# DredderGun/accbpg_and_fw

Hardware: AMD Instinct MI355X
Metric: D-opt iters/sec (m=2048,n=32768) (higher is better)
Workload: dtype f64; 1 GPU; D_opt_design(2048,32768) abpg_gain gamma=2 fp64, one independent instance per GPU; instances=1, instances_per_gpu=1, seeds=1..1, window=transient: iterations 5..161 from x0 = 1/n, linear_gram=False

## Files before the change

### accbpg_and_fw_amd/csrc/capi.hip

```cpp
#include <stdarg.h>
#include <string.h>
#include <stdlib.h>
#include <algorithm>

#include "internal.h"
#include "reduce.hpp"
#include "trial_verdict.h"

namespace accbpg {

static thread_local char g_err[512] = "";

void set_last_error(const char* fmt, ...) {
    va_list ap;
    va_start(ap, fmt);
    vsnprintf(g_err, sizeof(g_err), fmt, ap);
    va_end(ap);
}

void note_tiles_fallback(const char* where) {
    static bool said = false;
    if (said) return;
    said = true;
    fprintf(stderr, "libaccbpg_hip: %s: the one-launch Cholesky abandoned a wait (another process on this GPU, or fewer "
// ... 526 lines not shown
        return accbpg_dopt_eval_gram(h, gram_dev, flag, f_host, g_dev);
    }
    if (fl[FLAG_NOT_PD]) {
        set_last_error("HXHT is singular or not positive definite");
        return ACCBPG_ERR_NOT_PD;
    }
    if (f_host) *f_host = -h->hpin[0];
    return ACCBPG_OK;
}

extern "C" int accbpg_dopt_profile_enable(accbpg_dopt* h, int enable) {
    if (!h) return ACCBPG_ERR_ARG;
    h->prof_on = enable != 0;
    return ACCBPG_OK;
}

extern "C" int accbpg_dopt_profile_reset(accbpg_dopt* h) {
    if (!h) return ACCBPG_ERR_ARG;
    ACC_HIP(hipStreamSynchronize(h->stream));
    for (auto& p : h->prof) { p.used = 0; p.total_ms = 0.0; p.launches = 0; }
    return ACCBPG_OK;
}

extern "C" int accbpg_dopt_profile_read(accbpg_dopt* h, int which, double* total_ms_host, int64_t* launches_host) {
    if (!h || which < 0 || which >= PROF_COUNT) return ACCBPG_ERR_ARG;
    ACC_HIP(hipStreamSynchronize(h->stream));
    ProfSlot& p = h->prof[which];
    double tot = 0.0;
    for (size_t i = 0; i + 1 < p.used; i += 2) {
        float ms = 0.f;
        ACC_HIP(hipEventElapsedTime(&ms, p.ev[i], p.ev[i + 1]));
        tot += ms;
    }
    p.total_ms = tot;
    if (total_ms_host) *total_ms_host = tot;
    if (launches_host) *launches_host = p.launches;
    return ACCBPG_OK;
}

extern "C" int accbpg_mfma_f64_peak(int iters, double* tflops_host, void* stream) {
    if (!tflops_host || iters <= 0) return ACCBPG_ERR_ARG;
    return mfma_peak(iters, tflops_host, (hipStream_t)stream);
}

extern "C" int accbpg_debug_pipe_probe(int iters, int mode, double* ms_host, void* stream) {
    if (!ms_host || iters <= 0) return ACCBPG_ERR_ARG;
    return pipe_probe(iters, mode, ms_host, (hipStream_t)stream);
}

extern "C" int accbpg_test_gemm(const double* A_dev, int64_t lda, const double* B_dev, int64_t ldb, double* C_dev,
                                int64_t ldc, int64_t M, int64_t N, int64_t K, int b_kmajor, double alpha,
                                double beta, int config, void* stream) {
    if (!A_dev || !B_dev || !C_dev || M <= 0 || N <= 0 || K <= 0) return ACCBPG_ERR_ARG;
    return launch_test_gemm(A_dev, lda, B_dev, ldb, C_dev, ldc, M, N, K, b_kmajor, alpha, beta, config,
                            (hipStream_t)stream);
}

extern "C" int accbpg_dopt_factor_in_small_launches(accbpg_dopt* h, int on) {
    if (!h || on < 0 || on > 2) return ACCBPG_ERR_ARG;
    const int64_t T = (h->m + NB - 1) / NB;
    value_forget(h);
    h->chol_tiles_off = on == 1 || (on == 2 && T * (T + 1) / 2 >= h->num_cu);
    return ACCBPG_OK;
}

extern "C" int accbpg_debug_plan_flags(int flags) {
    set_plan_flags(flags);
    return ACCBPG_OK;
}

extern "C" int accbpg_debug_gemm_loop(int variant) {
    return set_gemm_loop(variant);
}

extern "C" int accbpg_debug_chol_variant(accbpg_dopt* h, int bits) {
    if (!h) return ACCBPG_ERR_ARG;
    value_forget(h);
    h->chol_dbg = bits & 63;
    h->chol_tiles_off = (bits & 64) != 0;
    if (bits & 2048) h->chol_tiles_off = true;
    h->chol_stall_test = (bits & 128) ? 1 : 0;
    h->chol_spin_limit = (bits & 128) ? 200000 : 20000000;
    h->kern_variant = (bits >> 30) & 3;
    if (bits & 256) h->use_glds = false;
    if (bits & 512) h->use_glds = true;
    if (bits & 2048) {
        h->chol_two_level_T = (bits >> 12) & 0xfff;
        if ((bits >> 24) & 0x3f) h->chol_nk = (bits >> 24) & 0x3f;
    }
    return ACCBPG_OK;
}

extern "C" int accbpg_debug_chol_trace(accbpg_dopt* h, const double* gram_dev, int with_inverse, int64_t* stamps_host) {
    if (!h || !gram_dev || !stamps_host) return ACCBPG_ERR_ARG;
    if (!chol_tiles_usable(h)) {
        set_last_error("accbpg_debug_chol_trace: the one-launch Cholesky is not in use for this handle");
        return ACCBPG_ERR_ARG;
    }
    const int T = (int)((h->m + NB - 1) / NB);
    const size_t bytes = sizeof(long long) * (size_t)T * 32;
    if (!h->chol_trace) ACC_HIP(acc_malloc(&h->chol_trace, bytes, "chol_trace"));
    ACC_HIP(hipMemsetAsync(h->chol_trace, 0, bytes, h->stream));
    int rc = launch_cholesky(h, h->Lbuf, with_inverse ? h->Wbuf : nullptr, nullptr, gram_dev);
    if (rc == ACCBPG_OK) {
        hipError_t e = hipMemcpyAsync(stamps_host, h->chol_trace, bytes, hipMemcpyDeviceToHost, h->stream);
        if (e == hipSuccess) e = hipStreamSynchronize(h->stream);
        if (e != hipSuccess) rc = ACCBPG_ERR_HIP;
    }
    acc_free(h->chol_trace);
    h->chol_trace = nullptr;
    return rc;
}

extern "C" int accbpg_debug_gram_variant(accbpg_dopt* h, const double* x_dev, int variant, int iters, double* ms_host) {
    if (!h || !x_dev || !ms_host || iters <= 0) return ACCBPG_ERR_ARG;
    value_forget(h);
    return debug_gram_variant(h, x_dev, variant, iters, ms_host);
}

extern "C" int accbpg_debug_grad_variant(accbpg_dopt* h, double* g_dev, int variant, int iters, double* ms_host) {
    if (!h || !g_dev || !ms_host || iters <= 0) return ACCBPG_ERR_ARG;
    value_forget(h);
    return debug_grad_variant(h, g_dev, variant, iters, ms_host);
}
```

### accbpg_and_fw_amd/csrc/dopt_kernels.hip

```cpp
#include <atomic>
#include <mutex>
#include <type_traits>

#include "internal.h"
#include "mfma_tile.hpp"

namespace accbpg {

struct GramSeg {
    int64_t row0, col0, kb, ke;
    bool dual, whole;
};
template <class T>
__device__ __forceinline__ GramSeg gram_segment(const TileRC* __restrict__ tiles, int64_t kiters, int64_t it,
                                                int64_t it1) {
    const int e = (int)(it / kiters);
    const int64_t off = it - (int64_t)e * kiters;
    const TileRC tr = tiles[e];
    GramSeg g;
    if (tr.d1 < 0) {
        g.row0 = (int64_t)tr.rb * T::BM; g.col0 = (int64_t)tr.cb * T::BN;
        g.kb = off; g.ke = min(kiters, off + (it1 - it));
        g.dual = false;
        g.whole = (g.kb == 0 && g.ke == kiters);
// ... 84 lines not shown
    }
}

template <class T, int GV = 0>
__device__ __forceinline__ void gram_streamk_glds_body(
    const double* __restrict__ V, int64_t ldv, int64_t m, int64_t n, const double* __restrict__ x,
    const TileRC* __restrict__ tiles, const int64_t* __restrict__ wg_ranges, int64_t kiters, int nslot,
    double* __restrict__ slabs,
    double* __restrict__ G, int64_t ldg, int all_slabs) {
    extern __shared__ __attribute__((aligned(16))) double lds[];
    constexpr int NLD = T::G_NA + T::G_NB + 1;
    T t;
    int seg = 0;
    for (int rg = 0; rg < GRAM_RMAX; ++rg) {
    int64_t it = wg_ranges[((int64_t)blockIdx.x * GRAM_RMAX + rg) * 2];
    const int64_t it1 = wg_ranges[((int64_t)blockIdx.x * GRAM_RMAX + rg) * 2 + 1];
    while (it < it1) {
        const GramSeg sg = gram_segment<T>(tiles, kiters, it, it1);
        const int64_t kb = sg.kb, ke = sg.ke, row0 = sg.row0, col0 = sg.col0;
        const int64_t klast = ke - 1;
        t.zero();
        if constexpr (T::WAVES_N == 1) {
            if (sg.dual) {
                constexpr int NLDD = T::G_NLD_DUAL;
                const int64_t khalf = (kiters >> 1) * BK;
                t.glds_setup_A_dual(V, ldv, row0, khalf);
                __builtin_amdgcn_s_barrier();
                t.glds_issue_dual(kb * BK, x, khalf, lds);
                t.glds_issue_dual(min(kb + 1, klast) * BK, x, khalf, lds + T::G_STAGE);
                asm volatile("s_waitcnt vmcnt(%0)" ::"n"(NLDD) : "memory");
                __builtin_amdgcn_s_barrier();
                int cur = 0;
                t.template read_frag_dual<0>(lds, 0);
#pragma unroll 1
                for (int64_t ks = kb; ks < ke; ++ks) {
                    int nx2 = cur + 2;
                    if (nx2 >= 3) nx2 -= 3;
                    const double* st = lds + cur * T::G_STAGE;
                    t.template scale_dual<0>();
                    __builtin_amdgcn_sched_barrier(0);
                    t.template read_frag_dual<1>(st, 1);
                    __builtin_amdgcn_sched_barrier(0);
                    t.template mma_dual<0>();
                    t.glds_issue_dual(min(ks + 2, klast) * BK, x, khalf, lds + nx2 * T::G_STAGE);
                    __builtin_amdgcn_sched_barrier(0);
                    t.template scale_dual<1>();
                    __builtin_amdgcn_sched_barrier(0);
                    t.template read_frag_dual<0>(st, 2);
                    __builtin_amdgcn_sched_barrier(0);
                    t.template mma_dual<1>();
                    __builtin_amdgcn_sched_barrier(0);
                    t.template scale_dual<0>();
                    __builtin_amdgcn_sched_barrier(0);
                    t.template read_frag_dual<1>(st, 3);
                    __builtin_amdgcn_sched_barrier(0);
                    t.template mma_dual<0>();
                    __builtin_amdgcn_sched_barrier(0);
                    t.template scale_dual<1>();
                    __builtin_amdgcn_sched_barrier(0);
                    asm volatile("s_waitcnt vmcnt(%0)\n\ts_waitcnt lgkmcnt(0)" ::"n"(NLDD) : "memory");
                    __builtin_amdgcn_s_barrier();
                    cur = (cur + 1 == 3) ? 0 : cur + 1;
                    t.template read_frag_dual<0>(lds + cur * T::G_STAGE, 0);
                    __builtin_amdgcn_sched_barrier(0);
                    t.template mma_dual<1>();
                    __builtin_amdgcn_sched_barrier(0);
                }
                asm volatile("s_waitcnt vmcnt(0)\n\ts_waitcnt lgkmcnt(0)" ::: "memory");
                t.store_slab(slabs + ((int64_t)blockIdx.x * nslot + seg) * T::SLAB_DOUBLES);
                it += ke - kb;
                ++seg;
                continue;
            }
        }
        constexpr int PAIR = (GV & 256) ? 4 : (GV & 128) ? 2 : 1;
        t.template glds_setup_A<PAIR>(V, ldv, row0);
        t.template glds_setup_B_kc<PAIR>(V, ldv, col0);
        auto issue = [&](int64_t ks, int buf) {
            double* st = lds + buf * T::G_STAGE;
            t.template glds_issue<PAIR>(ks * BK, ks * BK, st);
            t.glds_x(x, ks * BK, st);
        };
        __builtin_amdgcn_s_barrier();
        issue(kb, 0);
        issue(min(kb + 1, klast), 1);
        asm volatile("s_waitcnt vmcnt(%0)" ::"n"(NLD) : "memory");
        __builtin_amdgcn_s_barrier();
        int cur = 0;
        t.template read_frag_g<0, true>(lds, 0);
        static_assert(T::MI == 4, "group 0 is dealt out over four fragment rows");
        constexpr int NP = T::G_NA + T::G_NB;
        constexpr int P1 = (NP + 2) / 3, P2 = 2 * P1 < NP ? 2 * P1 : NP;
        if constexpr (GV & 32) {
#pragma unroll 1
            for (int64_t ks = kb; ks < ke; ++ks) {
                int nx2 = cur + 2;
                if (nx2 >= 3) nx2 -= 3;
                int nx1 = cur + 1;
                if (nx1 >= 3) nx1 -= 3;
                const double* st = lds + cur * T::G_STAGE;
                const double* st1 = lds + nx1 * T::G_STAGE;
                double* nst = lds + nx2 * T::G_STAGE;
                const int64_t k2 = min(ks + 2, klast) * BK;
                auto group = [&](auto gtag) {
                    constexpr int g = decltype(gtag)::value;
                    constexpr int S = g & 1, NS = S ^ 1;
                    static_for<0, 16>([&](auto qtag) {
                        constexpr int q = decltype(qtag)::value;
                        constexpr int I = q >> 2, P = q & 3;
                        if constexpr (P == 0) t.template scale_row<S, I>();
                        __builtin_amdgcn_sched_barrier(0);
                        constexpr bool PB = (GV & 64) != 0;
                        constexpr int QBAR = PB ? 4 : 8;
                        if constexpr (g == 3 && q == QBAR && !(GV & 2)) {
                            if constexpr (GV & 8) asm volatile("s_waitcnt lgkmcnt(0)" ::: "memory");
                            else asm volatile("s_waitcnt vmcnt(%0)\n\ts_waitcnt lgkmcnt(0)" ::"n"(NLD) : "memory");
                            __builtin_amdgcn_s_barrier();
                        }
                        t.template mma_pair<S, I, P>();
                        __builtin_amdgcn_sched_barrier(0);
                        if constexpr (g < 3) {
                            constexpr int rp = PB ? q - 1 : (((q & 1) == 1) ? (q >> 1) : -1);
                            if constexpr (rp >= 0 && rp < 7 && !(GV & 4)) t.template read_part_g<NS, true, rp>(st, g + 1);
                            constexpr int lp = PB ? q - 8 : (((q & 1) == 0) ? (q >> 1) : -1);
                            if constexpr (g == 0 && lp >= 0 && !(GV & 1)) {
                                constexpr int p0 = 2 * lp;
                                if constexpr (PAIR == 4) {
                                    if constexpr (p0 < NP && p0 % 4 == 0) t.template glds_issue_range<4>(k2, k2, nst, p0, p0 + 4);
                                } else if constexpr (p0 < NP) t.template glds_issue_range<PAIR>(k2, k2, nst, p0, p0 + 2 < NP ? p0 + 2 : NP);
                                if constexpr (p0 == NP || (p0 + 1 == NP)) t.glds_x(x, k2, nst);
                            }
                        } else {
                            constexpr int rp = q - QBAR - (PB ? 1 : 0);
                            if constexpr (rp >= 0 && rp < 7 && !(GV & 4)) t.template read_part_g<NS, true, rp>(st1, 0);
                        }
                        __builtin_amdgcn_sched_barrier(0);
                    });
                };
                group(std::integral_constant<int, 0>{});
                group(std::integral_constant<int, 1>{});
                group(std::integral_constant<int, 2>{});
                group(std::integral_constant<int, 3>{});
                cur = nx1;
            }
        } else {
#pragma unroll 1
        for (int64_t ks = kb; ks < ke; ++ks) {
            int nx2 = cur + 2;
            if (nx2 >= 3) nx2 -= 3;
            const double* st = lds + cur * T::G_STAGE;
            double* nst = lds + nx2 * T::G_STAGE;
            const int64_t k2 = min(ks + 2, klast) * BK;
            t.template scale_frag<0>();
            __builtin_amdgcn_sched_barrier(0);
            if constexpr (!(GV & 4)) t.template read_frag_g<1, true>(st, 1);
            __builtin_amdgcn_sched_barrier(0);
            t.template mma_row<0>(0);
            if constexpr (!(GV & 1)) t.glds_issue_range(k2, k2, nst, 0, P1);
            t.template mma_row<0>(1);
            if constexpr (!(GV & 1)) t.glds_issue_range(k2, k2, nst, P1, P2);
            t.template mma_row<0>(2);
            if constexpr (!(GV & 1)) { t.glds_issue_range(k2, k2, nst, P2, NP); t.glds_x(x, k2, nst); }
            t.template mma_row<0>(3);
            __builtin_amdgcn_sched_barrier(0);
            t.template scale_frag<1>();
            __builtin_amdgcn_sched_barrier(0);
            if constexpr (!(GV & 4) && !(GV & 16)) t.template read_frag_g<0, true>(st, 2);
            __builtin_amdgcn_sched_barrier(0);
            t.template mma_frag<1>();
            __builtin_amdgcn_sched_barrier(0);
            t.template scale_frag<0>();
            __builtin_amdgcn_sched_barrier(0);
            if constexpr (!(GV & 4)) t.template read_frag_g<1, true>(st, 3);
            __builtin_amdgcn_sched_barrier(0);
            t.template mma_frag<0>();
            __builtin_amdgcn_sched_barrier(0);
            t.template scale_frag<1>();
            __builtin_amdgcn_sched_barrier(0);
            if constexpr (!(GV & 2)) {
                if constexpr (GV & 8) asm volatile("s_waitcnt lgkmcnt(0)" ::: "memory");
                else asm volatile("s_waitcnt vmcnt(%0)\n\ts_waitcnt lgkmcnt(0)" ::"n"(NLD) : "memory");
                __builtin_amdgcn_s_barrier();
            }
            cur = (cur + 1 == 3) ? 0 : cur + 1;
            if constexpr (!(GV & 4) && !(GV & 16)) t.template read_frag_g<0, true>(lds + cur * T::G_STAGE, 0);
            __builtin_amdgcn_sched_barrier(0);
            t.template mma_frag<1>();
            __builtin_amdgcn_sched_barrier(0);
        }
        }
        asm volatile("s_waitcnt vmcnt(0)\n\ts_waitcnt lgkmcnt(0)" ::: "memory");
        if (sg.whole && !all_slabs) {
            t.store_C(G, ldg, row0, col0, m, m, 1.0, 0.0, true);
        } else {
            t.store_slab(slabs + ((int64_t)blockIdx.x * nslot + seg) * T::SLAB_DOUBLES);
        }
        it += ke - kb;
        ++seg;
    }
    }
}

constexpr int GRAM_GV = 224;
template <class T, int GV = 0>
__global__ __launch_bounds__(NTHREADS, 1) void gram_streamk_glds_kernel(
    const double* __restrict__ V, int64_t ldv, int64_t m, int64_t n, const double* __restrict__ x,
    const TileRC* __restrict__ tiles, const int64_t* __restrict__ wg_ranges, int64_t kiters, int nslot,
    double* __restrict__ slabs,
    double* __restrict__ G, int64_t ldg, int all_slabs) {
    gram_streamk_glds_body<T, GV>(V, ldv, m, n, x, tiles, wg_ranges, kiters, nslot, slabs, G, ldg, all_slabs);
}
template <class T>
__global__ __launch_bounds__(NTHREADS, 1) void gram_streamk_glds_batch_kernel(
    const BatchInst* __restrict__ bt, BatchAct act, int64_t ldv, int64_t m, int64_t n, const double* __restrict__ xbase,
    int64_t ldx, const TileRC* __restrict__ tiles, const int64_t* __restrict__ wg_ranges, int64_t kiters, int nslot,
    int64_t ldg) {
    const int inst = act.idx[blockIdx.y];
    const BatchInst bi = bt[inst];
    gram_streamk_glds_body<T, GRAM_GV>(bi.V, ldv, m, n, xbase + (int64_t)inst * ldx, tiles, wg_ranges, kiters, nslot, bi.slabs,
                                       bi.gram, ldg, 0);
}

constexpr int FIX_PJ = 4;
template <class T>
__device__ __forceinline__ void gram_fixup_body(
    const TileRC* __restrict__ tiles, const int32_t* __restrict__ cstart, const int32_t* __restrict__ contrib,
    int nslot, const double* __restrict__ slabs, double* __restrict__ G, int64_t ldg, int64_t m, double beta) {
    constexpr int JW = (T::NI + FIX_PJ - 1) / FIX_PJ;
    const int jq = blockIdx.x % FIX_PJ;
    const int b = blockIdx.x / FIX_PJ;
    const int e = b / (2 * T::MI), hs = (b / T::MI) & 1, part = b % T::MI;
    const int j0 = jq * JW, j1 = min(T::NI, j0 + JW);
    if (j0 >= T::NI) return;
    const TileRC tr = tiles[e];
    const bool dual = tr.d1 >= 0;
    if (dual && part >= T::MI / 2) return;
    const int c0 = cstart[2 * e + hs], c1 = cstart[2 * e + hs + 1];
    if (c0 == c1) return;
    int64_t row0 = (int64_t)tr.rb * T::BM, col0 = (int64_t)tr.cb * T::BN;
    if (dual) row0 = col0 = (int64_t)(hs ? tr.d2 : tr.d1) * (T::BM / 2);
    if (col0 + 16 * j0 > row0 + 16 * (part * T::WAVES_M + T::WAVES_M - 1) + 15) return;
    double a[JW][4];
#pragma unroll
    for (int jj = 0; jj < JW; ++jj)
#pragma unroll
        for (int r = 0; r < 4; ++r) a[jj][r] = 0.0;
    const int tid = threadIdx.x;
    for (int c = c0; c < c1; ++c) {
        const int64_t w = contrib[2 * c];
        const int slot = contrib[2 * c + 1];
        const double* sl = slabs + (w * nslot + slot) * T::SLAB_DOUBLES;
#pragma unroll
        for (int jj = 0; jj < JW; ++jj) {
            const int j = j0 + jj;
            if (j < j1) {
#pragma unroll
                for (int r = 0; r < 4; ++r) {
                    a[jj][r] += sl[((part * T::NI + j) * 4 + r) * NTHREADS + tid];
                    if (dual) a[jj][r] += sl[(((part + T::MI / 2) * T::NI + j) * 4 + r) * NTHREADS + tid];
                }
            }
        }
    }
    const int lane = tid & 63, wave = tid >> 6;
    const int wm = wave / T::WAVES_N, wn = wave % T::WAVES_N;
    const int lr = lane & 15, lq = lane >> 4;
#pragma unroll
    for (int jj = 0; jj < JW; ++jj) {
        const int j = j0 + jj;
        if (j < j1) {
#pragma unroll
            for (int r = 0; r < 4; ++r) {
                const int rblk = dual ? T::dual_row_block(part, wm) : part * T::WAVES_M + wm;
                const int64_t row = row0 + 16 * rblk + lq + 4 * r;
                const int64_t col = col0 + wn * T::WN + 16 * j + lr;
                if (row < m && col < m && col <= row) {
                    double* gp = G + row * ldg + col;
                    *gp = (beta != 0.0) ? a[jj][r] + beta * *gp : a[jj][r];
                }
            }
        }
    }
}

template <class T>
__global__ __launch_bounds__(NTHREADS, 2) void gram_fixup_kernel(
// ... 1770 lines not shown
int build_plans(accbpg_dopt* h) {
    const int64_t m = h->m;
    GramPlanIn in;
    in.m = m; in.n = h->n; in.ldv = h->ldv;
    in.big = h->big; in.vec_ok = h->vec_ok; in.use_glds = h->use_glds;
    in.num_cu = h->num_cu; in.grid_cap = h->gram_grid_cap; in.flags = g_plan_flags;
    const GramPlan gp = plan_gram(in);
    if (!gp.ok) return ACCBPG_ERR_ARG;
    h->gram_chunks = gp.chunks;
    h->gram_nc = gp.nc;
    h->kiters = gp.kiters;
    h->has_duals = gp.has_duals;
    h->ntiles = (int)gp.tiles.size();
    h->gram_grid = gp.grid;
    h->gram_per = gp.per;
    h->gram_nslot = gp.nslot;
    if (gp.want_block_copy) {
        const size_t bytes = sizeof(double) * (size_t)m * (size_t)h->n;
        if (acc_malloc(&h->Vblk, bytes, "Vblk") == hipSuccess) {
            for (int c = 0; c < gp.chunks; ++c)
                ACC_HIP(hipMemcpy2DAsync(h->Vblk + (size_t)c * m * gp.nc, sizeof(double) * gp.nc,
                                         h->V + (size_t)c * gp.nc, sizeof(double) * (size_t)h->ldv,
                                         sizeof(double) * gp.nc, (size_t)m, hipMemcpyDeviceToDevice, h->stream));
            ACC_HIP(hipStreamSynchronize(h->stream));
        } else {
            (void)hipGetLastError();
            h->Vblk = nullptr;
        }
    }
    ACC_TRY(upload(gp.tiles, &h->tiles, "tiles"));
    ACC_TRY(upload(gp.ranges, &h->wg_ranges, "wg_ranges"));
    ACC_TRY(upload(gp.cstart, &h->gram_cstart, "gram_cstart"));
    ACC_TRY(upload(gp.contrib, &h->gram_contrib, "gram_contrib"));
    const size_t tile_doubles = h->big ? (size_t)TILE_BIG_M * TILE_BIG_N : (size_t)TILE_SMALL_M * TILE_SMALL_N;
    ACC_HIP(acc_malloc(&h->slabs, sizeof(double) * (size_t)gp.grid * gp.nslot * tile_doubles, "slabs"));

    ACC_HIP(acc_malloc(&h->Pbuf, sizeof(double) * (size_t)m * m, "Pbuf"));
    MergePlan mp = plan_merges(m, h->Lbuf, h->Wbuf, h->Tbuf, h->Pbuf);
    h->ops_host = std::move(mp.ops);
    h->red_host = std::move(mp.reds);
    h->merge_stages = std::move(mp.stages);
    ACC_TRY(upload(h->ops_host, &h->ops, "ops"));
    ACC_TRY(upload(h->red_host, &h->red, "red"));
    const int T = (int)((m + NB - 1) / NB);
    ACC_HIP(acc_malloc(&h->chol_op, sizeof(GemmOp) * (size_t)(T + 1), "chol_op"));

    if (T <= CT_TMAX) {
        const std::vector<CholJob> jobs = chol_jobs(T);
        ACC_TRY(ensure_lds(h->device, reinterpret_cast<const void*>(chol_tiles_kernel), CT_LDS_BYTES));
        int per_cu = 0;
        ACC_HIP(hipOccupancyMaxActiveBlocksPerMultiprocessor(&per_cu, chol_tiles_kernel, NTHREADS, CT_LDS_BYTES));
        h->chol_tiles_grid = (int)jobs.size();
        h->chol_slots = std::min(per_cu, 2) * h->num_cu;
        h->chol_tiles_ok = per_cu >= 1 && (int64_t)jobs.size() <= (int64_t)h->chol_slots;
        if (h->chol_tiles_ok) {
            CholJob* jobs_dev = nullptr;
            ACC_TRY(upload(jobs, &jobs_dev, "chol_jobs"));
            h->chol_jobs = jobs_dev;
            ACC_HIP(acc_malloc(&h->chol_ready, sizeof(int) * (size_t)(T * T + 5 * T), "chol_ready"));
            ACC_HIP(hipMemsetAsync(h->chol_ready, 0, sizeof(int) * (size_t)(T * T + 5 * T), h->stream));
            ACC_HIP(acc_malloc(&h->chol_hand, sizeof(double) * (size_t)T * NB * NB, "chol_hand"));
            ACC_HIP(acc_malloc(&h->chol_aux, sizeof(double) * (size_t)T * CT_AUX, "chol_aux"));
            ACC_HIP(acc_malloc(&h->Gbuf, sizeof(double) * (size_t)m * m, "Gbuf"));
            ACC_HIP(hipMemsetAsync(h->Gbuf, 0, sizeof(double) * (size_t)m * m, h->stream));
        }
    }
    ACC_HIP(hipStreamSynchronize(h->stream));
    return ACCBPG_OK;
}

template <class T>
static int gram_launch_t(accbpg_dopt* h, const double* x, double* gram) {
    if constexpr (!T::EDGE && T::BM == 256) {
        if (h->use_glds || h->has_duals) {
            const int64_t nc = h->gram_chunks > 1 ? h->gram_nc : h->n;
            for (int c = 0; c < h->gram_chunks; ++c) {
                const double* Vc = h->Vblk ? h->Vblk + (int64_t)c * h->m * nc : h->V + (int64_t)c * nc;
                const int64_t ldc = h->Vblk ? nc : h->ldv;
                const double* xc = x + (int64_t)c * nc;
                const double beta = c == 0 ? 0.0 : 1.0;
                const int all_slabs = h->gram_chunks > 1 ? 1 : 0;
                prof_begin(h, PROF_GRAM);
#define ACC_GRAM_ARGS Vc, ldc, h->m, nc, xc, h->tiles, h->wg_ranges, h->kiters, h->gram_nslot, h->slabs, gram, h->m, all_slabs
                if (h->kern_variant == 1)
                    ACC_LAUNCH_LDS(h->device, (gram_streamk_glds_kernel<T, GRAM_GV ^ 128>), h->gram_grid, NTHREADS, T::G_LDS_BYTES, h->stream, ACC_GRAM_ARGS);
                else if (h->kern_variant == 3)
                    ACC_LAUNCH_LDS(h->device, (gram_streamk_glds_kernel<T, 0>), h->gram_grid, NTHREADS, T::G_LDS_BYTES, h->stream, ACC_GRAM_ARGS);
                else if (h->kern_variant == 2)
                    ACC_LAUNCH_LDS(h->device, (gram_streamk_glds_kernel<T, (GRAM_GV ^ 128) | 256>), h->gram_grid, NTHREADS, T::G_LDS_BYTES, h->stream, ACC_GRAM_ARGS);
                else
                    ACC_LAUNCH_LDS(h->device, (gram_streamk_glds_kernel<T, GRAM_GV>), h->gram_grid, NTHREADS, T::G_LDS_BYTES, h->stream, ACC_GRAM_ARGS);
#undef ACC_GRAM_ARGS
                ACC_HIP(hipGetLastError());
                prof_end(h, PROF_GRAM);
                prof_begin(h, PROF_GRAMFIX);
                gram_fixup_kernel<T><<<h->ntiles * 2 * T::MI * FIX_PJ, NTHREADS, 0, h->stream>>>(
                    h->tiles, h->gram_cstart, h->gram_contrib, h->gram_nslot, h->slabs, gram, h->m, h->m, beta);
                prof_end(h, PROF_GRAMFIX);
            }
            return ACCBPG_OK;
        }
    }
    prof_begin(h, PROF_GRAM);
    ACC_LAUNCH_LDS(h->device, gram_streamk_kernel<T>, h->gram_grid, NTHREADS, T::LDS_BYTES, h->stream,
        h->V, h->ldv, h->m, h->n, x, h->tiles, h->wg_ranges, h->kiters, h->gram_nslot, h->slabs, gram, h->m, h->vec_ok);
    ACC_HIP(hipGetLastError());
    prof_end(h, PROF_GRAM);
    prof_begin(h, PROF_GRAMFIX);
    gram_fixup_kernel<T><<<h->ntiles * 2 * T::MI * FIX_PJ, NTHREADS, 0, h->stream>>>(h->tiles, h->gram_cstart, h->gram_contrib, h->gram_nslot,
                                                                h->slabs, gram, h->m, h->m, 0.0);
    prof_end(h, PROF_GRAMFIX);
    return ACCBPG_OK;
}

template <class F>
static int timed_launches(hipStream_t s, int iters, double* ms_out, F&& launch) {
    hipEvent_t a, b;
    ACC_HIP(hipEventCreate(&a));
    if (hipEventCreate(&b) != hipSuccess) {
        hipEventDestroy(a);
        return ACCBPG_ERR_HIP;
    }
    auto timed = [&]() -> int {
        ACC_TRY(launch());
        ACC_HIP(hipEventRecord(a, s));
        for (int i = 0; i < iters; ++i) ACC_TRY(launch());
        ACC_HIP(hipEventRecord(b, s));
        ACC_HIP(hipEventSynchronize(b));
        float ms = 0.f;
        ACC_HIP(hipEventElapsedTime(&ms, a, b));
        *ms_out = ms / iters;
        ACC_HIP(hipGetLastError());
        return ACCBPG_OK;
    };
    const int rc = timed();
    hipEventDestroy(a);
    hipEventDestroy(b);
    return rc;
}

int debug_gram_variant(accbpg_dopt* h, const double* x, int var, int iters, double* ms_out) {
    using T = TileBig<false, false>;
    if (!h->big) return ACCBPG_ERR_ARG;
    if (h->has_duals && var < 10) return ACCBPG_ERR_ARG;
    auto launch = [&]() -> int {
#define ACC_LAUNCH_VAR(VV)                                                                                       \
    ACC_LAUNCH_LDS(h->device, (gram_streamk_kernel<T, VV>), h->gram_grid, NTHREADS, T::LDS_BYTES, h->stream,      \
        h->V, h->ldv, h->m, h->n, x, h->tiles, h->wg_ranges, h->kiters, h->gram_nslot, h->slabs, h->Tbuf, h->m, h->vec_ok)
#define ACC_LAUNCH_G(GG)                                                                                         \
    ACC_LAUNCH_LDS(h->device, (gram_streamk_glds_kernel<T, GG>), h->gram_grid, NTHREADS, T::G_LDS_BYTES, h->stream,          \
        h->V, h->ldv, h->m, h->n, x, h->tiles, h->wg_ranges, h->kiters, h->gram_nslot, h->slabs, h->Tbuf, h->m, 0)
        switch (var) {
            case 10: ACC_LAUNCH_G(0); break;
            case 11: ACC_LAUNCH_G(1); break;
            case 12: ACC_LAUNCH_G(2); break;
            case 13: ACC_LAUNCH_G(3); break;
            case 14: ACC_LAUNCH_G(4); break;
            case 15: ACC_LAUNCH_G(8); break;
            case 16: ACC_LAUNCH_G(7); break;
            case 17: ACC_LAUNCH_G(16); break;
            case 18: ACC_LAUNCH_G(32); break;
            case 19: ACC_LAUNCH_G(96); break;
            case 20: ACC_LAUNCH_G(97); break;
            case 21: ACC_LAUNCH_G(98); break;
            case 22: ACC_LAUNCH_G(100); break;
            case 23: ACC_LAUNCH_G(104); break;
            case 24: ACC_LAUNCH_G(103); break;
            case 25: ACC_LAUNCH_G(102); break;
            case 26: ACC_LAUNCH_G(101); break;
            case 27: ACC_LAUNCH_G(99); break;
            case 28: ACC_LAUNCH_G(224); break;
            case 29: ACC_LAUNCH_G(352); break;
            case 0: ACC_LAUNCH_VAR(0); break;
            case 1: ACC_LAUNCH_VAR(1); break;
            case 2: ACC_LAUNCH_VAR(2); break;
            case 3: ACC_LAUNCH_VAR(3); break;
            default: ACC_LAUNCH_VAR(4); break;
        }
#undef ACC_LAUNCH_VAR
        return ACCBPG_OK;
    };
    return timed_launches(h->stream, iters, ms_out, launch);
}

int launch_gram(accbpg_dopt* h, const double* x, double* gram) {
    bool xal = (reinterpret_cast<uintptr_t>(x) & 15) == 0;
    if (!xal && (h->has_duals || h->gram_chunks > 1)) {
        if (!h->xbuf) ACC_HIP(acc_malloc(&h->xbuf, sizeof(double) * (size_t)h->n, "xbuf"));
        ACC_TRY(device_copy(h->xbuf, x, (size_t)h->n, h->stream));
        x = h->xbuf;
        xal = true;
    }
    if (h->big) {
        const bool interior = h->vec_ok && xal && (h->m % 256 == 0) && (h->n % BK == 0);
        if (interior) ACC_TRY((gram_launch_t<TileBig<false, false>>(h, x, gram)));
        else ACC_TRY((gram_launch_t<TileBig<false, true>>(h, x, gram)));
    } else {
        const bool interior = h->vec_ok && xal && (h->m % 64 == 0) && (h->n % BK == 0);
        if (interior) ACC_TRY((gram_launch_t<TileSmall<false, false>>(h, x, gram)));
        else ACC_TRY((gram_launch_t<TileSmall<false, true>>(h, x, gram)));
    }
    ACC_HIP(hipGetLastError());
    return ACCBPG_OK;
}

__global__ __launch_bounds__(256) void copy_kernel(double* __restrict__ dst, const double* __restrict__ src, size_t n) {
    const size_t stride = (size_t)gridDim.x * 256;
    for (size_t i = (size_t)blockIdx.x * 256 + threadIdx.x; i < n; i += stride) dst[i] = src[i];
}
int device_copy(double* dst, const double* src, size_t ndoubles, hipStream_t s) {
    if (ndoubles == 0 || dst == src) return ACCBPG_OK;
    size_t nb = (ndoubles + 255) / 256;
    if (nb > 4096) nb = 4096;
    copy_kernel<<<(unsigned)nb, 256, 0, s>>>(dst, src, ndoubles);
    ACC_HIP(hipGetLastError());
    return ACCBPG_OK;
}

int launch_gemm_ops(const GemmOp* ops_dev, int nops, int maxM, int maxN, bool b_kmajor, hipStream_t s) {
    if (nops <= 0 || maxM <= 0 || maxN <= 0) return ACCBPG_OK;
    dim3 grid((maxN + 63) / 64, (maxM + 63) / 64, nops);
    int dev = 0;
    ACC_HIP(hipGetDevice(&dev));
    return with_gemm_loop([&](auto loop) -> int {
        constexpr int LOOP = decltype(loop)::value;
        if (b_kmajor)
            ACC_LAUNCH_LDS(dev, (gemm_ops_kernel<TileSmall<true>, LOOP>), grid, NTHREADS, TileSmall<true>::LDS_BYTES, s, ops_dev);
        else
            ACC_LAUNCH_LDS(dev, (gemm_ops_kernel<TileSmall<false>, LOOP>), grid, NTHREADS, TileSmall<false>::LDS_BYTES, s, ops_dev);
        ACC_HIP(hipGetLastError());
        return ACCBPG_OK;
    });
}

static std::mutex g_tiles_mu;
constexpr int TILES_RING = 16;
struct TilesRing {
    hipEvent_t ev[TILES_RING] = {};
    hipStream_t stream[TILES_RING] = {};
    int grid[TILES_RING] = {};
    long long issued = 0;
};
static TilesRing g_tiles[64];

bool chol_tiles_usable(const accbpg_dopt* h) {
    return h->chol_tiles_ok && !h->chol_tiles_off && (h->chol_dbg & 63) == 0;
}

static int launch_chol_tiles(accbpg_dopt* h, const double* src, double* A, double* Winv, double* dscal, int* dflag) {
    const int64_t m = h->m;
    const int T = (int)((m + NB - 1) / NB);
    CholInst ci;
    ci.src = src; ci.L = A; ci.Ldiag = h->Tbuf; ci.Winv = Winv; ci.logdet = dscal; ci.flags = dflag;
    ci.ready = h->chol_ready; ci.aux = h->chol_aux; ci.hand = h->chol_hand; ci.trace = h->chol_trace;
    const int dev = (h->device >= 0 && h->device < 64) ? h->device : 0;
// ... 326 lines not shown
```

### accbpg_and_fw_amd/csrc/internal.h

```cpp
#pragma once
#include <hip/hip_runtime.h>
#include <stdint.h>
#include <stdio.h>
#include <map>
#include <mutex>
#include <utility>
#include <vector>

#include "../../include/accbpg_hip.h"
#include "dopt_plan.hpp"

namespace accbpg {

void set_last_error(const char* fmt, ...);
void note_tiles_fallback(const char* where);

hipError_t acc_malloc(void** p, size_t bytes, const char* label);
hipError_t acc_free(void* p);
template <class T>
inline hipError_t acc_malloc(T** p, size_t bytes, const char* label) {
    return acc_malloc(reinterpret_cast<void**>(p), bytes, label);
}

#define ACC_HIP(call)                                                                         \
// ... 163 lines not shown
constexpr int STATUS_DOUBLES = 20;
constexpr int ACCBPG_RETRY = 100;

enum ProfKind { PROF_GRAM = 0, PROF_CHOL = 1, PROF_TRTRI = 2, PROF_GRAD = 3, PROF_GRAMFIX = 4, PROF_FWV = 5, PROF_COUNT = 6 };

struct ProfSlot {
    std::vector<hipEvent_t> ev;
    size_t used = 0;
    double total_ms = 0.0;
    int64_t launches = 0;
};

}

struct accbpg_dopt {
    const double* V = nullptr;
    int64_t m = 0, n = 0, ldv = 0;
    hipStream_t stream = nullptr;
    int device = 0;
    int num_cu = 256;
    bool big = false;
    bool force_big = false;
    int gram_grid_cap = 0;
    double* dscal_ext = nullptr;
    bool vec_ok = false;

    double* Lbuf = nullptr;
    double* Wbuf = nullptr;
    double* Tbuf = nullptr;
    double* slabs = nullptr;
    accbpg::TileRC* tiles = nullptr;
    int64_t* wg_ranges = nullptr;
    int32_t* gram_cstart = nullptr;
    int32_t* gram_contrib = nullptr;
    int ntiles = 0, gram_grid = 0, gram_per = 0, gram_nslot = 2;
    int64_t kiters = 0;
    int gram_chunks = 1;
    int64_t gram_nc = 0;
    double* Vblk = nullptr;
    double* dscal = nullptr;
    int* dflag = nullptr;
    double* hpin = nullptr;
    double* vws = nullptr;
    double* xbuf = nullptr;

    accbpg::GemmOp* ops = nullptr;
    std::vector<accbpg::GemmOp> ops_host;
    std::vector<accbpg::RedOp> red_host;
    using MergeStage = accbpg::MergeStage;
    std::vector<MergeStage> merge_stages;
    accbpg::RedOp* red = nullptr;
    double* Pbuf = nullptr;
    accbpg::GemmOp* chol_op = nullptr;

    double *fw_x = nullptr, *fw_w = nullptr, *fw_H = nullptr, *fw_hv = nullptr;
    double* fw_hpin_dev = nullptr;
    accbpg::FwInst fw{};
    bool fw_ready = false;
    struct FwSlot {
        accbpg_dopt* aux = nullptr;
        hipStream_t stream = nullptr;
        hipEvent_t ev_snap = nullptr;
        bool pending = false;
    };
    std::vector<FwSlot> fw_ring;
    int fw_ring_depth = 1;
    int fw_ring_small = 2;
    long long fw_ring_issued = 0, fw_ring_collected = 0;
    int fw_part_nblk = 0;
    bool fw_part_away = false;
    accbpg::FwRunSlot* fw_run = nullptr;
    accbpg_fw_step* fw_steps_pin = nullptr;
    accbpg_fw_step* fw_steps_dev = nullptr;
    double* fw_div_ws = nullptr;
    double* fw_div_pin = nullptr;
    double* fw_div_pin_dev = nullptr;
    int64_t fw_div_i = -1;
    accbpg::FwDivRunSlot* fw_div_run = nullptr;
    accbpg_fw_div_step* fw_div_steps_pin = nullptr;
    accbpg_fw_div_step* fw_div_steps_dev = nullptr;

    bool use_glds = true;
    int kern_variant = 0;
    bool diag_inv_ready = false;
    bool has_duals = false;
    int chol_nk = 8;
    int chol_two_level_T = 64;
    int chol_dbg = 0;
    bool chol_tiles_ok = false;
    bool chol_tiles_off = false;
    int chol_stall_test = 0;
    long long chol_spin_limit = 20000000;
    int chol_tiles_grid = 0;
    int chol_slots = 0;
    void* chol_jobs = nullptr;
    int* chol_ready = nullptr;
    double* chol_aux = nullptr;
    double* chol_hand = nullptr;
    long long* chol_trace = nullptr;
    double* Gbuf = nullptr;
    const double* last_x = nullptr;
    double* last_g = nullptr;
    int last_flag = 0;
    hipEvent_t ev_done = nullptr;
    bool val_reuse = true;
    bool val_valid = false;
    bool val_pending = false;
    bool val_hit = false;
    const double* val_x = nullptr;
    double* val_copy = nullptr;
    double val_f = 0.0;
    double val_answer = 0.0;
    int val_gen = 0;
    int64_t val_compares = 0, val_answered = 0;
    double* trial_stat = nullptr;
    double* trial_pin = nullptr;
    accbpg_dopt* val_peer = nullptr;
    std::vector<accbpg_dopt*> val_linked;
    bool prof_on = false;
    accbpg::ProfSlot prof[accbpg::PROF_COUNT];
};

struct accbpg_dopt_batch {
    int K = 0;
    std::vector<accbpg_dopt*> inst;
    hipStream_t stream = nullptr;
    int device = 0;
    bool fast = false;
    int chunk = 0;
    accbpg::BatchInst* table = nullptr;
    accbpg::CholInst* chol_table[2] = {nullptr, nullptr};
    accbpg::GemmOp* ops_all = nullptr;
    accbpg::RedOp* red_all = nullptr;
    int ops_per_inst = 0, red_per_inst = 0;
    double* dscal_all = nullptr;
    double* hpin = nullptr;
    int* vflags = nullptr;
    double* vout = nullptr;
    double* vpart = nullptr;
    double* vws = nullptr;
    double* vquot = nullptr;
    double* vpin = nullptr;
    accbpg::FwInst* fw_table = nullptr;
    accbpg::FwDivInst* fw_div_table = nullptr;
    accbpg::FwRunSlot* fw_runs = nullptr;
    accbpg_fw_step* fw_bsteps_pin = nullptr;
    accbpg_fw_step* fw_bsteps_dev = nullptr;
    accbpg::FwDivRunSlot* fw_div_runs = nullptr;
    accbpg_fw_div_step* fw_div_bsteps_pin = nullptr;
    accbpg_fw_div_step* fw_div_bsteps_dev = nullptr;
    accbpg::BatchAct pend_act;
    const double* pend_x = nullptr;
    double* pend_g = nullptr;
    int64_t pend_ldx = 0, pend_ldg = 0;
    int pend_flag = 0;
    bool pend_fused = false;
};
struct BatchVals { double v[accbpg::BATCH_MAX]; };

namespace accbpg {

int launch_gram_batch(accbpg_dopt_batch* b, const BatchAct& act, const double* xbase, int64_t ldx);
int launch_cholesky_batch(accbpg_dopt_batch* b, const BatchAct& act, bool with_inverse, const double* xbase, int64_t ldx);
int launch_trtri_batch(accbpg_dopt_batch* b, const BatchAct& act);
int launch_colnorm_batch(accbpg_dopt_batch* b, const BatchAct& act, double* gbase, int64_t ldg, double sign);

// ... 44 lines not shown
```

### accbpg_and_fw_amd/csrc/mfma_tile.hpp

```cpp
#pragma once
#include <hip/hip_runtime.h>
#include <stdint.h>
#include <type_traits>

#include "dopt_plan.hpp"

namespace accbpg {

typedef double d4 __attribute__((ext_vector_type(4)));
typedef double d2 __attribute__((ext_vector_type(2)));

constexpr int SK = BK + 2;
constexpr int NTHREADS = 256;

typedef const __attribute__((address_space(1))) double* gptr;
__device__ __forceinline__ gptr as_global(const double* p) { return (gptr)p; }
__device__ __forceinline__ d2 ld2(const double* p) { return *reinterpret_cast<const d2*>(p); }
__device__ __forceinline__ d2 ld2(gptr p) { return *(const __attribute__((address_space(1))) d2*)p; }

template <class P>
__device__ __forceinline__ d2 load2_guard(P p, bool row_ok, int64_t k, int64_t K, bool vec_ok) {
    d2 v;
    if (row_ok && vec_ok && k + 1 < K) {
        v = ld2(p);
// ... 320 lines not shown
                        constexpr int pb = p - G_NA;
                        if constexpr (NPK == 2) glds16_run2<pb * 1024>(bb, gob[pb], gob[pb + 1], lb);
                        else glds16_run4<pb * 1024>(bb, gob[pb], gob[pb + 1], gob[pb + 2], gob[pb + 3], lb);
                    }
                }
            });
            return;
        }
#pragma unroll
        for (int p = 0; p < G_NA + G_NB; ++p)
            if (p >= p0 && p < p1) {
                uint32_t o = (p < G_NA) ? goa[p < G_NA ? p : 0] : gob[p >= G_NA ? p - G_NA : 0];
                asm volatile("" : "+v"(o));
                const char* b = (p < G_NA) ? ba : bb;
                glds16(reinterpret_cast<const double*>(b + o), stage + (p < G_NA ? 0 : G_A) + (wave + 4 * (p < G_NA ? p : p - G_NA)) * 128);
            }
    }
    __device__ __forceinline__ void glds_x(const double* __restrict__ x, int64_t k0, double* __restrict__ stage) const {
        const int lane = threadIdx.x & 63;
        const float* src = reinterpret_cast<const float*>(x + k0) + (lane & 31);
        __builtin_amdgcn_global_load_lds((const __attribute__((address_space(1))) void*)src,
                                         (__attribute__((address_space(3))) void*)(stage + G_A + G_B), 4, 0, 0);
    }
    template <int SET, bool SCALE>
    __device__ __forceinline__ void read_frag_g(const double* __restrict__ stage, int kk) {
        const int lane = threadIdx.x & 63, wave = __builtin_amdgcn_readfirstlane(threadIdx.x >> 6);
        const int wm = wave / WAVES_N, wn = wave % WAVES_N;
        const int lr = lane & 15, lq = lane >> 4;
        const int sw = (lr >> 1) & 7;
        const int koff = 2 * ((2 * kk + (lq >> 1)) ^ sw) + (lq & 1);
        const double* as = stage + (16 * wm + lr) * BK + koff;
#pragma unroll
        for (int i = 0; i < MI; ++i) fa[SET][i] = as[i * 16 * WAVES_M * BK];
        if constexpr (BKM) {
            const double* bs = stage + G_A + (4 * kk + lq) * BN + wn * WN + lr;
#pragma unroll
            for (int j = 0; j < NI; ++j) fb[SET][j] = bs[16 * (j ^ (lq & 1))];
        } else {
            const double* bs = stage + G_A + (wn * WN + lr) * BK + koff;
#pragma unroll
            for (int j = 0; j < NI; ++j) fb[SET][j] = bs[j * 16 * BK];
        }
        if constexpr (SCALE) fx[SET] = stage[G_A + G_B + 4 * kk + lq];
    }

    template <int SET, bool SCALE, int PART>
    __device__ __forceinline__ void read_part_g(const double* __restrict__ stage, int kk) {
        static_assert(MI == 4 && NI == 8, "parts are laid out for the 64 x 128 wave tile");
        const int lane = threadIdx.x & 63, wave = __builtin_amdgcn_readfirstlane(threadIdx.x >> 6);
        const int wm = wave / WAVES_N, wn = wave % WAVES_N;
        const int lr = lane & 15, lq = lane >> 4;
        const int sw = (lr >> 1) & 7;
        const int koff = 2 * ((2 * kk + (lq >> 1)) ^ sw) + (lq & 1);
        if constexpr (PART == 0) {
            if constexpr (SCALE) fx[SET] = stage[G_A + G_B + 4 * kk + lq];
        } else if constexpr (PART == 1 || PART == 6) {
            const double* as = stage + (16 * wm + lr) * BK + koff;
            constexpr int i0 = (PART == 1) ? 0 : 2;
            fa[SET][i0] = as[i0 * 16 * WAVES_M * BK];
            fa[SET][i0 + 1] = as[(i0 + 1) * 16 * WAVES_M * BK];
        } else {
            constexpr int j0 = 2 * (PART - 2);
            if constexpr (BKM) {
                const double* bs = stage + G_A + (4 * kk + lq) * BN + wn * WN + lr;
                fb[SET][j0] = bs[16 * (j0 ^ (lq & 1))];
                fb[SET][j0 + 1] = bs[16 * ((j0 + 1) ^ (lq & 1))];
            } else {
                const double* bs = stage + G_A + (wn * WN + lr) * BK + koff;
                fb[SET][j0] = bs[j0 * 16 * BK];
                fb[SET][j0 + 1] = bs[(j0 + 1) * 16 * BK];
            }
        }
    }
    template <int SET, int I>
    __device__ __forceinline__ void scale_row() { fa[SET][I] *= fx[SET]; }
    template <int SET, int I, int P>
    __device__ __forceinline__ void mma_pair(int mi_lo = 0) {
        if (I >= mi_lo) {
            acc[I][2 * P] = __builtin_amdgcn_mfma_f64_16x16x4f64(fa[SET][I], fb[SET][2 * P], acc[I][2 * P], 0, 0, 0);
            acc[I][2 * P + 1] = __builtin_amdgcn_mfma_f64_16x16x4f64(fa[SET][I], fb[SET][2 * P + 1], acc[I][2 * P + 1], 0, 0, 0);
        }
    }

    template <int SET, int ILO>
    __device__ __forceinline__ void read_frag_lo(const double* __restrict__ stage, int kk) {
        static_assert(BKM, "the gradient product reads a k-major B image");
        const int lane = threadIdx.x & 63, wave = __builtin_amdgcn_readfirstlane(threadIdx.x >> 6);
        const int wm = wave / WAVES_N, wn = wave % WAVES_N;
        const int lr = lane & 15, lq = lane >> 4;
        const int sw = (lr >> 1) & 7;
        const int koff = 2 * ((2 * kk + (lq >> 1)) ^ sw) + (lq & 1);
        const double* as = stage + (16 * wm + lr) * BK + koff;
#pragma unroll
        for (int i = ILO; i < MI; ++i) fa[SET][i] = as[i * 16 * WAVES_M * BK];
        const double* bs = stage + G_A + (4 * kk + lq) * BN + wn * WN + lr;
#pragma unroll
        for (int j = 0; j < NI; ++j) fb[SET][j] = bs[16 * (j ^ (lq & 1))];
    }
    template <int SET, int I, int ILO, bool COND>
    __device__ __forceinline__ void mma_row_lo(bool live) {
        if constexpr (I >= ILO) {
            if (!(COND && I == ILO) || live) {
#pragma unroll
                for (int j = 0; j < NI; ++j)
                    acc[I][j] = __builtin_amdgcn_mfma_f64_16x16x4f64(fa[SET][I], fb[SET][j], acc[I][j], 0, 0, 0);
            }
        }
    }
    template <int SET, int ILO, bool COND>
    __device__ __forceinline__ void mma_frag_lo(bool live) {
        static_assert(MI == 4, "four fragment rows");
        mma_row_lo<SET, 0, ILO, COND>(live);
        mma_row_lo<SET, 1, ILO, COND>(live);
        mma_row_lo<SET, 2, ILO, COND>(live);
        mma_row_lo<SET, 3, ILO, COND>(live);
    }
    template <int RUN, int ILO, int ILO_NEXT, bool COND, int NLD, int AB = 0>
    __device__ __forceinline__ void grad_step(const double* __restrict__ st, const double* __restrict__ st1,
                                              double* __restrict__ nst, int64_t ka, int64_t kb, bool live) {
        constexpr int NP = G_NA + G_NB;
        constexpr int P1 = (NP + 2) / 3, P2 = 2 * P1 < NP ? 2 * P1 : NP;
        static_assert(NLD == NP, "every wave retires the loads of one step per step");
        if constexpr (!(AB & 4)) read_frag_lo<1, ILO>(st, 1);
        __builtin_amdgcn_sched_barrier(0);
        mma_row_lo<0, 0, ILO, COND>(live);
        if constexpr (!(AB & 1)) glds_issue_range<RUN>(ka, kb, nst, 0, P1);
        mma_row_lo<0, 1, ILO, COND>(live);
        if constexpr (!(AB & 1)) glds_issue_range<RUN>(ka, kb, nst, P1, P2);
        mma_row_lo<0, 2, ILO, COND>(live);
        if constexpr (!(AB & 1)) glds_issue_range<RUN>(ka, kb, nst, P2, NP);
        mma_row_lo<0, 3, ILO, COND>(live);
        __builtin_amdgcn_sched_barrier(0);
        if constexpr (!(AB & 4)) read_frag_lo<0, ILO>(st, 2);
        __builtin_amdgcn_sched_barrier(0);
        mma_frag_lo<1, ILO, COND>(live);
        __builtin_amdgcn_sched_barrier(0);
        if constexpr (!(AB & 4)) read_frag_lo<1, ILO>(st, 3);
        __builtin_amdgcn_sched_barrier(0);
        mma_frag_lo<0, ILO, COND>(live);
        __builtin_amdgcn_sched_barrier(0);
        if constexpr (!(AB & 2)) {
            asm volatile("s_waitcnt vmcnt(%0)\n\ts_waitcnt lgkmcnt(0)" ::"n"(NLD) : "memory");
            __builtin_amdgcn_s_barrier();
        }
        if constexpr (!(AB & 4)) read_frag_lo<0, ILO_NEXT>(st1, 0);
        __builtin_amdgcn_sched_barrier(0);
        mma_frag_lo<1, ILO, COND>(live);
        __builtin_amdgcn_sched_barrier(0);
    }

    static constexpr int DEALT_PART_VALUES = 2;
    template <int SET, int PART, int ILO>
    __device__ __forceinline__ void read_part_lo(const double* __restrict__ stage, int kk) {
        if constexpr (PART == 1 || PART == 6) {
            const int lane = threadIdx.x & 63, wave = __builtin_amdgcn_readfirstlane(threadIdx.x >> 6);
            const int wm = wave / WAVES_N;
            const int lr = lane & 15, lq = lane >> 4;
            const int sw = (lr >> 1) & 7;
            const int koff = 2 * ((2 * kk + (lq >> 1)) ^ sw) + (lq & 1);
            const double* as = stage + (16 * wm + lr) * BK + koff;
            constexpr int i0 = (PART == 1) ? 0 : 2;
            if constexpr (i0 >= ILO) fa[SET][i0] = as[i0 * 16 * WAVES_M * BK];
            if constexpr (i0 + 1 >= ILO) fa[SET][i0 + 1] = as[(i0 + 1) * 16 * WAVES_M * BK];
        } else {
            read_part_g<SET, false, PART>(stage, kk);
        }
// ... 270 lines not shown
```

Before: 66.35 iterations/s.

## Unroll Gram stream-K main loop by three stages with constant LDS addresses

Adds a Gram kernel variant (GV bit 512) whose k-loop is unrolled over the three LDS pipeline stages. Stage indices, LDS fragment addresses and global-to-LDS source pointers become compile-time constants or precomputed registers, which removes the per-iteration modular stage arithmetic and address recomputation. The remainder iterations are peeled, and waitcnt/barrier placement is hand-scheduled. The variant becomes the default, and the old rolled loop stays reachable through a debug flag. In exchange, the kernel has much more code and higher register pressure from the precomputed address arrays.

New measurement: 68.69 iterations/s (median of 6 runs). 3.5% higher.

```diff
diff --git a/accbpg_and_fw_amd/csrc/capi.hip b/accbpg_and_fw_amd/csrc/capi.hip
--- a/accbpg_and_fw_amd/csrc/capi.hip
+++ b/accbpg_and_fw_amd/csrc/capi.hip
@@ -632,6 +632,7 @@
     h->chol_stall_test = (bits & 128) ? 1 : 0;
     h->chol_spin_limit = (bits & 128) ? 200000 : 20000000;
     h->kern_variant = (bits >> 30) & 3;
+    h->gram_rolled = (bits & 1024) ? 1 : 0;
     if (bits & 256) h->use_glds = false;
     if (bits & 512) h->use_glds = true;
     if (bits & 2048) {
diff --git a/accbpg_and_fw_amd/csrc/dopt_kernels.hip b/accbpg_and_fw_amd/csrc/dopt_kernels.hip
--- a/accbpg_and_fw_amd/csrc/dopt_kernels.hip
+++ b/accbpg_and_fw_amd/csrc/dopt_kernels.hip
@@ -190,8 +190,19 @@
             t.glds_x(x, ks * BK, st);
         };
         __builtin_amdgcn_s_barrier();
-        issue(kb, 0);
-        issue(min(kb + 1, klast), 1);
+        if constexpr (GV & 512) {
+            const int64_t k1 = min(kb + 1, klast);
+            t.frag_setup(lds);
+            t.glds_src(x, (int)kb);
+            t.template glds_issue<PAIR>(kb * BK, kb * BK, lds);
+            t.template glds_x_c<0>();
+            t.glds_src(x, (int)k1);
+            t.template glds_issue<PAIR>(k1 * BK, k1 * BK, lds + T::G_STAGE);
+            t.template glds_x_c<1>();
+        } else {
+            issue(kb, 0);
+            issue(min(kb + 1, klast), 1);
+        }
         asm volatile("s_waitcnt vmcnt(%0)" ::"n"(NLD) : "memory");
         __builtin_amdgcn_s_barrier();
         int cur = 0;
@@ -199,7 +210,87 @@
         static_assert(T::MI == 4, "group 0 is dealt out over four fragment rows");
         constexpr int NP = T::G_NA + T::G_NB;
         constexpr int P1 = (NP + 2) / 3, P2 = 2 * P1 < NP ? 2 * P1 : NP;
-        if constexpr (GV & 32) {
+        if constexpr (GV & 512) {
+            static_assert((GV & 32) && (GV & 64) && PAIR == 2, "the constant-stage loop is the production schedule");
+            constexpr int QBAR = 4;
+            const int L = (int)(ke - kb);
+            int trips = (L > 2 ? L - 2 : 0) / 3;
+            asm volatile("" : "+s"(trips));
+            auto step = [&](auto ctag, auto atag) {
+                constexpr int CUR = decltype(ctag)::value, NX1 = (CUR + 1) % 3, NX2 = (CUR + 2) % 3;
+                constexpr bool ADV = decltype(atag)::value;
+                static_for<0, 4>([&](auto gtag) {
+                    constexpr int g = decltype(gtag)::value;
+                    constexpr int S = g & 1, NS = S ^ 1;
+                    static_for<0, 16>([&](auto qtag) {
+                        constexpr int q = decltype(qtag)::value;
+                        constexpr int I = q >> 2, P = q & 3;
+                        if constexpr (P == 3 && I < 3) t.template scale_row<S, I + 1>();
+                        if constexpr (P == 3 && I == 3) {
+                            __builtin_amdgcn_s_waitcnt(0xC07F);
+                            __builtin_amdgcn_sched_barrier(0);
+                            t.template scale_row<NS, 0>();
+                        }
+                        __builtin_amdgcn_sched_barrier(0);
+                        if constexpr (g == 3 && q == QBAR && !(GV & 2)) {
+                            asm volatile("s_waitcnt vmcnt(%0)\n\ts_waitcnt lgkmcnt(0)" ::"n"(NLD) : "memory");
+                            __builtin_amdgcn_s_barrier();
+                        }
+                        t.template mma_pair<S, I, P>();
+                        __builtin_amdgcn_sched_barrier(0);
+                        if constexpr (g < 3) {
+                            constexpr int rp = q - 1;
+                            if constexpr (rp >= 0 && rp < 7 && !(GV & 4)) t.template read_part_c<NS, rp, CUR, g + 1>();
+                            constexpr int p0 = 2 * (q - 8);
+                            if constexpr (g == 0 && p0 >= 0 && !(GV & 1)) {
+                                if constexpr (p0 < NP) t.template glds_pair_c<NX2, p0>();
+                                if constexpr (p0 == NP) {
+                                    t.template glds_x_c<NX2>();
+                                    if constexpr (ADV) t.glds_src_advance();
+                                }
+                            }
+                        } else {
+                            constexpr int rp = q - QBAR - 1;
+                            if constexpr (rp >= 0 && rp < 7 && !(GV & 4)) t.template read_part_c<NS, rp, NX1, 0>();
+                        }
+                        __builtin_amdgcn_sched_barrier(0);
+                    });
+                });
+            };
+            constexpr std::integral_constant<int, 0> s0{};
+            constexpr std::integral_constant<int, 1> s1{};
+            constexpr std::integral_constant<int, 2> s2{};
+            t.template scale_row<0, 0>();
+            t.glds_src(x, (int)kb + 2);
+#pragma unroll 1
+            for (int tr = 0; tr < trips; ++tr) {
+                t.pin_acc();
+                step(s0, std::true_type{});
+                step(s1, std::true_type{});
+                step(s2, std::true_type{});
+            }
+            t.pin_acc();
+            const int rest = L - 3 * trips;
+            const int kt = (int)kb + 3 * trips + 2, kl = (int)klast;
+            t.glds_src(x, min(kt, kl));
+            step(s0, std::false_type{});
+            t.pin_acc();
+            if (rest >= 2) {
+                t.glds_src(x, min(kt + 1, kl));
+                step(s1, std::false_type{});
+                t.pin_acc();
+                if (rest >= 3) {
+                    t.glds_src(x, min(kt + 2, kl));
+                    step(s2, std::false_type{});
+                    t.pin_acc();
+                    if (rest >= 4) {
+                        t.glds_src(x, min(kt + 3, kl));
+                        step(s0, std::false_type{});
+                        t.pin_acc();
+                    }
+                }
+            }
+        } else if constexpr (GV & 32) {
 #pragma unroll 1
             for (int64_t ks = kb; ks < ke; ++ks) {
                 int nx2 = cur + 2;
@@ -309,7 +400,8 @@
     }
 }
 
-constexpr int GRAM_GV = 224;
+constexpr int GRAM_GV = 224 | 512;
+constexpr int GRAM_GV_ROLLED = 224;
 template <class T, int GV = 0>
 __global__ __launch_bounds__(NTHREADS, 1) void gram_streamk_glds_kernel(
     const double* __restrict__ V, int64_t ldv, int64_t m, int64_t n, const double* __restrict__ x,
@@ -2246,12 +2338,14 @@
                 const int all_slabs = h->gram_chunks > 1 ? 1 : 0;
                 prof_begin(h, PROF_GRAM);
 #define ACC_GRAM_ARGS Vc, ldc, h->m, nc, xc, h->tiles, h->wg_ranges, h->kiters, h->gram_nslot, h->slabs, gram, h->m, all_slabs
-                if (h->kern_variant == 1)
-                    ACC_LAUNCH_LDS(h->device, (gram_streamk_glds_kernel<T, GRAM_GV ^ 128>), h->gram_grid, NTHREADS, T::G_LDS_BYTES, h->stream, ACC_GRAM_ARGS);
+                if (h->gram_rolled && h->kern_variant == 0)
+                    ACC_LAUNCH_LDS(h->device, (gram_streamk_glds_kernel<T, GRAM_GV_ROLLED>), h->gram_grid, NTHREADS, T::G_LDS_BYTES, h->stream, ACC_GRAM_ARGS);
+                else if (h->kern_variant == 1)
+                    ACC_LAUNCH_LDS(h->device, (gram_streamk_glds_kernel<T, GRAM_GV_ROLLED ^ 128>), h->gram_grid, NTHREADS, T::G_LDS_BYTES, h->stream, ACC_GRAM_ARGS);
                 else if (h->kern_variant == 3)
                     ACC_LAUNCH_LDS(h->device, (gram_streamk_glds_kernel<T, 0>), h->gram_grid, NTHREADS, T::G_LDS_BYTES, h->stream, ACC_GRAM_ARGS);
                 else if (h->kern_variant == 2)
-                    ACC_LAUNCH_LDS(h->device, (gram_streamk_glds_kernel<T, (GRAM_GV ^ 128) | 256>), h->gram_grid, NTHREADS, T::G_LDS_BYTES, h->stream, ACC_GRAM_ARGS);
+                    ACC_LAUNCH_LDS(h->device, (gram_streamk_glds_kernel<T, (GRAM_GV_ROLLED ^ 128) | 256>), h->gram_grid, NTHREADS, T::G_LDS_BYTES, h->stream, ACC_GRAM_ARGS);
                 else
                     ACC_LAUNCH_LDS(h->device, (gram_streamk_glds_kernel<T, GRAM_GV>), h->gram_grid, NTHREADS, T::G_LDS_BYTES, h->stream, ACC_GRAM_ARGS);
 #undef ACC_GRAM_ARGS
@@ -2335,6 +2429,13 @@
             case 27: ACC_LAUNCH_G(99); break;
             case 28: ACC_LAUNCH_G(224); break;
             case 29: ACC_LAUNCH_G(352); break;
+            case 30: ACC_LAUNCH_G(736); break;
+            case 31: ACC_LAUNCH_G(742); break;
+            case 32: ACC_LAUNCH_G(739); break;
+            case 33: ACC_LAUNCH_G(743); break;
+            case 34: ACC_LAUNCH_G(230); break;
+            case 35: ACC_LAUNCH_G(227); break;
+            case 36: ACC_LAUNCH_G(231); break;
             case 0: ACC_LAUNCH_VAR(0); break;
             case 1: ACC_LAUNCH_VAR(1); break;
             case 2: ACC_LAUNCH_VAR(2); break;
diff --git a/accbpg_and_fw_amd/csrc/internal.h b/accbpg_and_fw_amd/csrc/internal.h
--- a/accbpg_and_fw_amd/csrc/internal.h
+++ b/accbpg_and_fw_amd/csrc/internal.h
@@ -269,6 +269,7 @@
 
     bool use_glds = true;
     int kern_variant = 0;
+    int gram_rolled = 0;
     bool diag_inv_ready = false;
     bool has_duals = false;
     int chol_nk = 8;
diff --git a/accbpg_and_fw_amd/csrc/mfma_tile.hpp b/accbpg_and_fw_amd/csrc/mfma_tile.hpp
--- a/accbpg_and_fw_amd/csrc/mfma_tile.hpp
+++ b/accbpg_and_fw_amd/csrc/mfma_tile.hpp
@@ -426,6 +426,89 @@
         }
     }
 
+    typedef const __attribute__((address_space(3))) double* lptr;
+    uint32_t fra[3][4], frb[3][4], frx[3];
+    uint32_t gla, glb, glx, gxo;
+    const char* gpa;
+    const char* gpb;
+    const char* gpx;
+    __device__ __forceinline__ void frag_setup(const double* __restrict__ lds) {
+        static_assert(!BKM, "k-contiguous B image");
+        const int lane = threadIdx.x & 63, wave = __builtin_amdgcn_readfirstlane(threadIdx.x >> 6);
+        const int wm = wave / WAVES_N, wn = wave % WAVES_N;
+        const int lr = lane & 15, lq = lane >> 4;
+        const int sw = (lr >> 1) & 7;
+#pragma unroll
+        for (int s = 0; s < 3; ++s) {
+            const double* stage = lds + s * G_STAGE;
+#pragma unroll
+            for (int kk = 0; kk < 4; ++kk) {
+                const int koff = 2 * ((2 * kk + (lq >> 1)) ^ sw) + (lq & 1);
+                fra[s][kk] = lds_addr(stage + (16 * wm + lr) * BK + koff);
+                frb[s][kk] = lds_addr(stage + G_A + (wn * WN + lr) * BK + koff);
+                asm volatile("" : "+v"(fra[s][kk]));
+                asm volatile("" : "+v"(frb[s][kk]));
+            }
+            frx[s] = lds_addr(stage + G_A + G_B + lq);
+            asm volatile("" : "+v"(frx[s]));
+        }
+        gla = lds_addr(lds + wave * G_NA * 128);
+        glb = lds_addr(lds + G_A + wave * G_NB * 128);
+        glx = lds_addr(lds + G_A + G_B);
+        gxo = (uint32_t)(lane & 31) * 4;
+        asm volatile("" : "+s"(gla));
+        asm volatile("" : "+s"(glb));
+        asm volatile("" : "+s"(glx));
+        asm volatile("" : "+v"(gxo));
+    }
+    __device__ __forceinline__ void glds_src(const double* __restrict__ x, int k) {
+        gpa = gbase_a + (int64_t)k * (BK * 8);
+        gpb = gbase_b + (int64_t)k * (BK * 8);
+        gpx = reinterpret_cast<const char*>(x) + (int64_t)k * (BK * 8);
+        asm volatile("" : "+s"(gpa));
+        asm volatile("" : "+s"(gpb));
+        asm volatile("" : "+s"(gpx));
+    }
+    __device__ __forceinline__ void glds_src_advance() {
+        gpa += BK * 8;
+        gpb += BK * 8;
+        gpx += BK * 8;
+        asm volatile("" : "+s"(gpa));
+        asm volatile("" : "+s"(gpb));
+        asm volatile("" : "+s"(gpx));
+    }
+    template <int STG, int P0>
+    __device__ __forceinline__ void glds_pair_c() const {
+        static_assert(G_NA % 2 == 0 && G_NB % 2 == 0 && P0 % 2 == 0 && P0 < G_NA + G_NB, "whole runs of two");
+        if constexpr (P0 < G_NA) glds16_run2<STG * G_STAGE * 8 + P0 * 1024>(gpa, goa[P0], goa[P0 + 1], gla);
+        else glds16_run2<STG * G_STAGE * 8 + (P0 - G_NA) * 1024>(gpb, gob[P0 - G_NA], gob[P0 - G_NA + 1], glb);
+    }
+#pragma clang diagnostic push
+#pragma clang diagnostic ignored "-Winline-asm"
+    template <int STG>
+    __device__ __forceinline__ void glds_x_c() const {
+        asm volatile("s_add_u32 m0, %2, %3\n\ts_nop 0\n\tglobal_load_lds_dword %0, %1"
+                     :: "v"(gxo), "s"(gpx), "s"(glx), "i"(STG * G_STAGE * 8) : "memory", "scc", "m0");
+    }
+#pragma clang diagnostic pop
+    template <int SET, int PART, int STG, int KK>
+    __device__ __forceinline__ void read_part_c() {
+        static_assert(MI == 4 && NI == 8, "parts are laid out for the 64 x 128 wave tile");
+        if constexpr (PART == 0) {
+            fx[SET] = reinterpret_cast<lptr>(frx[STG])[4 * KK];
+        } else if constexpr (PART == 1 || PART == 6) {
+            lptr as = reinterpret_cast<lptr>(fra[STG][KK]);
+            constexpr int i0 = (PART == 1) ? 0 : 2;
+            fa[SET][i0] = as[i0 * 16 * WAVES_M * BK];
+            fa[SET][i0 + 1] = as[(i0 + 1) * 16 * WAVES_M * BK];
+        } else {
+            lptr bs = reinterpret_cast<lptr>(frb[STG][KK]);
+            constexpr int j0 = 2 * (PART - 2);
+            fb[SET][j0] = bs[j0 * 16 * BK];
+            fb[SET][j0 + 1] = bs[(j0 + 1) * 16 * BK];
+        }
+    }
+
     template <int SET, int ILO>
     __device__ __forceinline__ void read_frag_lo(const double* __restrict__ stage, int kk) {
         static_assert(BKM, "the gradient product reads a k-major B image");
```
